# NVIDIA-Merlin/NVTabular

Hardware: AMD Instinct MI355X
Metric: rows/sec + GB/s (Criteo Categorify+FillMissing+Normalize fit+transform, HBM-resident) (higher is better)
Workload: dtype int32 keys -> int64 labels; fp64 moments/normalize; 1 GPU; synthetic Criteo-day0: 26 int32 categorical (Criteo-1TB cardinalities, Zipf) + 13 int32 continuous, nulls as Arrow bitmaps; Categorify + FillMissing + Normalize, fit + transform; rows_per_gpu=45000000, algorithmic_bytes_per_row=624, tie_break=value (count desc, value asc), artifacts=deferred (no parquet I/O inside the timed region)

## Files before the change

nvtabular_amd/csrc/nvt_range_count.hip:

```cpp
#include <cstdio>
#include <cstdlib>
#include <type_traits>

#include "nvt_common.hpp"
#include "nvt_internal.hpp"
#include "nvt_prof.hpp"
#include "nvt_range.hpp"

namespace nvt {

namespace {

constexpr int32_t kEmpty = INT32_MIN;
constexpr int kRpBS = 1024;
constexpr int kRpG = NVT_RANGE_WGS;
constexpr int kRpBinWords = 20480;
constexpr int kRpLine = 16;
constexpr int kRpMaxNbLog2 = 10;
constexpr int kHotSlotsR = NVT_HOT_IMAGE_WORDS;
constexpr int kHotBucketsR = kHotSlotsR / 2;
constexpr int kRpProbe = 512;
#ifndef NVT_RP_MAX_EPOCH
#define NVT_RP_MAX_EPOCH 8
#endif
constexpr unsigned kRpMaxEpoch = NVT_RP_MAX_EPOCH;
#ifndef NVT_RANGE_U
#define NVT_RANGE_U 2
#endif
constexpr unsigned long long kStAgg = 1ull << 62, kStPrefix = 2ull << 62,
                             kStMask = (1ull << 62) - 1ull;

__device__ __forceinline__ uint32_t hot_bucket_r(int32_t key) { return hot_image_bucket(key, kHotBucketsR - 1); }

template <bool PW>
__device__ __forceinline__ uint32_t rp_fine(const RangeMap &map, int32_t key) {
  if constexpr (PW) return map.fine(key);
  else return map.template fine_staged<false>(key);
}


template <int U, int NBL, bool PW>
__global__ __launch_bounds__(kRpBS) void rp_partition_kernel(
    const int32_t *__restrict__ keys, const uint8_t *__restrict__ valid, uint64_t n,
    const int32_t *__restrict__ aux, int nb_log2_rt, uint32_t region_cap, int32_t *__restrict__ regions,
    uint32_t *__restrict__ fills, unsigned *__restrict__ hot_cnt, uint64_t *state,
    unsigned long long *__restrict__ clr_status, unsigned *__restrict__ clr_hist) {
  const int nb_log2 = NBL ? NBL : nb_log2_rt;
  {
    const unsigned nst = (1u << nb_log2) + 8u;
    for (unsigned i = blockIdx.x * kRpBS + threadIdx.x; i < nst; i += kRpG * kRpBS) clr_status[i] = 0ull;
    if (blockIdx.x == kRpG - 1 && threadIdx.x < 256) clr_hist[threadIdx.x] = 0u;
  }
  __shared__ int4 hot[kHotBucketsR];
  __shared__ int32_t bins[kRpBinWords];
  __shared__ unsigned fill[1 << kRpMaxNbLog2], flushed[1 << kRpMaxNbLog2];
  __shared__ unsigned scratch[kWave];
  __shared__ unsigned long long s_nulls, s_sent;
  __shared__ unsigned s_ovf;
  const unsigned NB = 1u << nb_log2, CAP = (unsigned)kRpBinWords >> nb_log2;
  const unsigned g = blockIdx.x, lane = lane_id();
  int32_t fill0 = 0x5A5A5A5A, fill1 = fill0 + 1;
  while (hot_bucket_r(fill1) == hot_bucket_r(fill0)) ++fill1;
  const uint32_t fb0 = hot_bucket_r(fill0);
  for (int i = threadIdx.x; i < kHotBucketsR; i += kRpBS) {
    const int2 k2 = reinterpret_cast<const int2 *>(aux)[i];
    const int32_t fk = (uint32_t)i != fb0 ? fill0 : fill1;
    hot[i] = make_int4(k2.x == kEmpty ? fk : k2.x, k2.y == kEmpty ? fk : k2.y, 0, 0);
  }
  for (unsigned i = threadIdx.x; i < NB; i += kRpBS) {
    fill[i] = 0;
    flushed[i] = 0;
  }
  if (threadIdx.x == 0) {
    s_nulls = 0;
    s_sent = 0;
    s_ovf = 0;
  }
  RangeMap map = load_map(aux);
  __shared__ uint32_t s_pieces[kRpPwWords];
  stage_pieces(map, s_pieces, threadIdx.x, kRpBS);
  __syncthreads();

  const unsigned BPW = NB / (kRpBS / kWave);
  __shared__ unsigned s_epoch[2];
  if (threadIdx.x < 2) s_epoch[threadIdx.x] = 0;
  auto flush_bins = [&](bool all, unsigned parity) {
    {
      const bool owner = lane < BPW;
      const unsigned wave_base = (threadIdx.x / kWave) * BPW;
      const unsigned t = wave_base + (owner ? lane : 0u);
      const unsigned fr = owner ? fill[t] : 0u;
      const unsigned done0 = owner ? flushed[t] : 0u;
      const bool over = fr > CAP;
      const unsigned f = over ? CAP : fr;
      const unsigned nfl = (all || over) ? f : (f / kRpLine) * kRpLine;
      const unsigned padn = over ? ((0u - (done0 + fr)) & (kRpLine - 1u)) : 0u;
      {
        const unsigned long long ob = __ballot(over);
        const unsigned long long hb = __ballot(fr * 2u > CAP);
        if (lane == 0 && (ob | hb))
          atomicAdd(&s_epoch[parity], ((unsigned)__popcll(ob) << 8) | (hb ? 1u : 0u));
      }
      unsigned long long todo = __ballot(nfl > 0);
      const unsigned sub = lane >> 4, l16 = lane & 15;
      while (todo) {
        int sel = -1;
#pragma unroll
        for (unsigned q = 0; q < 4; ++q) {
          const int bit = todo ? (int)__ffsll((long long)todo) - 1 : -1;
          if (todo) todo &= todo - 1;
          sel = (q == sub) ? bit : sel;
        }
        const unsigned src = sel >= 0 ? (unsigned)sel : 0u;
        const unsigned fb = __shfl(f, src, 64), nb_out = __shfl(nfl, src, 64);
        const unsigned done = __shfl(done0, src, 64), frb = __shfl(fr, src, 64), pb = __shfl(padn, src, 64);
        if (sel >= 0) {
          const unsigned bin = wave_base + (unsigned)sel;
          const int32_t *bsrc = bins + bin * CAP;
          const unsigned reach = frb > fb ? done + frb + pb : done + nb_out;
          if (reach > region_cap) {
            if (l16 == 0) atomicOr(&s_ovf, 1u);
          } else {
            int32_t *dst = regions + ((uint64_t)bin * kRpG + g) * region_cap + done;
            for (unsigned u = l16; u < nb_out; u += kRpLine) dst[u] = bsrc[u];
            if (l16 < pb) dst[frb + l16] = kEmpty;
          }
          const unsigned rem = fb - nb_out;
          int32_t keep = 0;
          if (l16 < rem) keep = bsrc[nb_out + l16];
          if (l16 < rem) bins[bin * CAP + l16] = keep;
        }
      }
      if (owner) {
        fill[t] = f - nfl;
        flushed[t] = over ? done0 + fr + padn : done0 + nfl;
      }
    }
  };

  const uint64_t nvec = (n + 3) / 4, nfull = n / 4;
  const uint64_t per = (nvec + kRpG - 1) / kRpG;
  const uint64_t v_lo = (uint64_t)g * per;
  const uint64_t v_hi = v_lo + per < nvec ? v_lo + per : nvec;
  const uint64_t vf_hi = v_hi < nfull ? v_hi : nfull;
  unsigned long long nulls = 0, notvalid = 0;
  unsigned long long empties = 0;
  const uint8_t *vsrc = valid != nullptr ? valid : reinterpret_cast<const uint8_t *>(keys);
  const unsigned vor = valid != nullptr ? 0u : 0xFFu;
  const uint64_t v_last = vf_hi > v_lo ? vf_hi - 1 : 0;
  int4 npack[U];
  unsigned nbyte[U];
  auto issue = [&](uint64_t v0) {
#pragma unroll
    for (int u = 0; u < U; ++u) {
      uint64_t v = v0 + (uint64_t)u * kRpBS;
      v = v < v_last ? v : v_last;
      npack[u] = reinterpret_cast<const int4 *>(keys)[v];
      nbyte[u] = (unsigned)vsrc[v >> 1];
    }
  };
  bool tail_round = false;
  int4 tpack = make_int4(0, 0, 0, 0);
  unsigned tok = 0, tin = 0;
  if (nfull < nvec && nfull >= v_lo && nfull < v_hi) {
    tail_round = true;
    if (threadIdx.x == 0) {
      int32_t kk[4] = {0, 0, 0, 0};
      for (int j = 0; j < 4; ++j) {
        const uint64_t i = nfull * 4 + j;
        if (i < n) {
          tin |= 1u << j;
          if (bit_valid(valid, i)) {
            kk[j] = keys[i];
            tok |= 1u << j;
          }
        }
      }
      tpack = make_int4(kk[0], kk[1], kk[2], kk[3]);
    }
  }
  unsigned R = 1, since = 0, epoch = 0;
  if (vf_hi > v_lo) issue(v_lo + threadIdx.x);
  for (uint64_t v0 = v_lo; v0 < vf_hi || tail_round; v0 += (uint64_t)kRpBS * U) {
    const bool is_tail = !(v0 < vf_hi);
    int32_t kv[4 * U];
    unsigned oks[U], ins[U];
#pragma unroll
    for (int u = 0; u < U; ++u) {
      const uint64_t v = v0 + (uint64_t)u * kRpBS + threadIdx.x;
      const bool present = !is_tail && v < vf_hi;
      kv[4 * u + 0] = npack[u].x;
      kv[4 * u + 1] = npack[u].y;
      kv[4 * u + 2] = npack[u].z;
      kv[4 * u + 3] = npack[u].w;
      oks[u] = present ? (((nbyte[u] | vor) >> (((unsigned)v & 1u) * 4u)) & 0xFu) : 0u;
      ins[u] = present ? 0xFu : 0u;
    }
    if (is_tail) {
      tail_round = false;
      kv[0] = tpack.x;
      kv[1] = tpack.y;
      kv[2] = tpack.z;
      kv[3] = tpack.w;
      oks[0] = tok;
      ins[0] = tin;
    } else {
      issue(v0 + (uint64_t)kRpBS * U + threadIdx.x);
    }
    unsigned pend = 0;
#pragma unroll
    for (int u = 0; u < U; ++u) {
      const unsigned ok = oks[u], in = ins[u];
      nulls += __popc(in & ~ok);
      notvalid += 4u - __popc(ok);
      int32_t kp[4];
      int4 hb[4];
      uint32_t sa[4];
#pragma unroll
      for (int j = 0; j < 4; ++j) {
        const int32_t m = (int32_t)(ok << (31 - j)) >> 31;
        kp[j] = (kv[4 * u + j] & m) | (kEmpty & ~m);
        sa[j] = hot_bucket_r(kp[j]);
      }
#pragma unroll
      for (int j = 0; j < 4; ++j) {
        const int2 kk2 = *reinterpret_cast<const int2 *>(&hot[sa[j]]);
        hb[j].x = kk2.x;
        hb[j].y = kk2.y;
      }
#pragma unroll
      for (int j = 0; j < 4; ++j) {
        const int q = 4 * u + j;
        const int32_t key = kp[j];
        const bool hx = hb[j].x == key, hy = hb[j].y == key;
        const bool hit = hx | hy;
        const bool is_e = key == kEmpty;
        empties += (unsigned)__popcll(__ballot(is_e));
        unsigned *cnt = reinterpret_cast<unsigned *>(&hot[sa[j]]) + (hy ? 3 : 2);
        atomicAdd(hit ? cnt : &scratch[lane], hit ? 1u : 0u);
        pend |= ((!hit & !is_e) ? 1u : 0u) << q;
      }
    }
    if (s_ovf) pend = 0;
#pragma unroll
    for (int q = 0; q < 4 * U; ++q) {
      if ((pend >> q) & 1) {
        const unsigned bkt = rp_fine<PW>(map, kv[q]) >> 14;
        const unsigned pos = atomicAdd(&fill[bkt], 1u);
        if (pos < CAP) {
          bins[bkt * CAP + pos] = kv[q];
        } else {
          const unsigned at = flushed[bkt] + pos;
          if (at < region_cap)
            regions[((uint64_t)bkt * kRpG + g) * region_cap + at] = kv[q];
          else
            atomicOr(&s_ovf, 1u);
        }
      }
    }
    if (++since >= R) {
      __syncthreads();
      flush_bins(false, epoch & 1u);
      if (threadIdx.x == 0) s_epoch[(epoch + 1u) & 1u] = 0;
      __syncthreads();
      const unsigned fl = s_epoch[epoch & 1u];
#ifndef NVT_RP_GROW_DIV
#define NVT_RP_GROW_DIV 16u
#endif
#ifndef NVT_RP_SHRINK_DIV
#define NVT_RP_SHRINK_DIV 4u
#endif
      if ((fl >> 8) > NB / NVT_RP_SHRINK_DIV) R = R > 1u ? R / 2u : 1u;
      else if ((fl >> 8) <= NB / NVT_RP_GROW_DIV) R = R < kRpMaxEpoch ? R * 2u : R;
      ++epoch;
      since = 0;
    }
  }
  __syncthreads();
  flush_bins(true, epoch & 1u);
  __syncthreads();
  for (unsigned b = threadIdx.x; b < NB; b += kRpBS) fills[(uint64_t)b * kRpG + g] = flushed[b];
  for (int i = threadIdx.x; i < kHotBucketsR; i += kRpBS) {
    const int4 hbk = hot[i];
    reinterpret_cast<uint2 *>(hot_cnt + (uint64_t)g * kHotSlotsR)[i] = make_uint2((unsigned)hbk.z, (unsigned)hbk.w);
  }
#pragma unroll
  for (int off = 32; off > 0; off >>= 1) {
    nulls += __shfl_down(nulls, off, 64);
    notvalid += __shfl_down(notvalid, off, 64);
  }
  if (lane == 0) {
    if (nulls) atomicAdd(&s_nulls, nulls);
    const unsigned long long sent = empties - notvalid;
    if (sent) atomicAdd(&s_sent, sent);
  }
  __syncthreads();
  if (threadIdx.x == 0) {
    if (s_nulls) atomicAdd((unsigned long long *)&state[NVT_ST_NULLS], s_nulls);
    if (s_sent) atomicAdd((unsigned long long *)&state[NVT_ST_SENTINEL], s_sent);
    if (s_ovf) atomicOr((unsigned long long *)&state[NVT_ST_OVERFLOW], 1ull | NVT_OVF_REGION);
    if (g == 0) atomicAdd((unsigned long long *)&state[NVT_ST_ROWS], (unsigned long long)n);
  }
}

constexpr int kTotGroups = 16;
__global__ __launch_bounds__(64 * kTotGroups) void hot_totals_kernel(
    const unsigned *__restrict__ hot_cnt, int nblocks, unsigned *__restrict__ hot_tot) {
  __shared__ unsigned part[kTotGroups][64];
  const unsigned l = threadIdx.x & 63, g = threadIdx.x >> 6;
  const unsigned slot = blockIdx.x * 64 + l;
  unsigned t = 0;
#pragma unroll 16
  for (int b = (int)g; b < nblocks; b += kTotGroups) t += hot_cnt[(uint64_t)b * kHotSlotsR + slot];
  part[g][l] = t;
  __syncthreads();
  if (g != 0) return;
  unsigned tot = 0;
#pragma unroll
  for (int q = 0; q < kTotGroups; ++q) tot += part[q][l];
  hot_tot[slot] = tot;
}

template <bool PW>
__global__ __launch_bounds__(kRpBS) void rp_count_kernel(
    const int32_t *__restrict__ regions, const uint32_t *__restrict__ fills, uint32_t region_cap,
    const int32_t *__restrict__ aux, const unsigned *__restrict__ hot_tot, int nb_log2,
    unsigned long long *status, unsigned *ticket, int32_t *__restrict__ out_keys,
    int64_t *__restrict__ out_cnt, uint64_t out_cap, unsigned *cls_hist,
    unsigned long long *__restrict__ range_table, uint64_t *state) {
  constexpr int NSL = kRpSlots + kRpTail;
  constexpr int NW = kRpBS / kWave;
  __shared__ int32_t lkeys[NSL];
  __shared__ unsigned lcnt[NSL];
  __shared__ unsigned run_len[kRpG];
  __shared__ unsigned hist[256];
  __shared__ unsigned wtot[NW];
  __shared__ unsigned lovf, s_b, s_bad, s_mx;
  __shared__ unsigned long long s_base;
  if (threadIdx.x == 0) {
    s_b = atomicAdd(ticket, 1u);
    lovf = 0;
    s_mx = 0;
  }
  for (int i = threadIdx.x; i < NSL; i += kRpBS) {
    lkeys[i] = kEmpty;
    lcnt[i] = 0;
  }
  if (threadIdx.x < 256) hist[threadIdx.x] = 0;
  __syncthreads();
  const unsigned b = s_b, NB = 1u << nb_log2;
  const unsigned lane = lane_id(), w = threadIdx.x / kWave;
  RangeMap map = load_map(aux);
  __shared__ uint32_t s_pieces[kRpPwWords];
  stage_pieces(map, s_pieces, threadIdx.x, kRpBS);
  const bool skip = (state[NVT_ST_OVERFLOW] & 1ull) != 0;
  if (threadIdx.x < kRpG) {
    const unsigned len = fills[(uint64_t)b * kRpG + threadIdx.x];
    run_len[threadIdx.x] = (skip || len > region_cap) ? 0u : len;
  }
  __syncthreads();
  bool failed = skip;
  auto insert_from = [&](int32_t key, unsigned wgt, uint32_t s) {
#pragma unroll 4
    for (int p = 0; p < kRpProbe; ++p, ++s) {
      if (s >= (uint32_t)NSL) break;
      int32_t cur = lkeys[s];
      if (cur == kEmpty) {
        cur = atomicCAS(&lkeys[s], kEmpty, key);
        if (cur == kEmpty) cur = key;
      }
      if (cur == key) {
        atomicAdd(&lcnt[s], wgt);
        return;
      }
    }
    failed = true;
  };
  const unsigned hot_h0 = (unsigned)aux[NVT_RANGE_AUX_HOTSTART + b], hot_h1 = (unsigned)aux[NVT_RANGE_AUX_HOTSTART + b + 1];
  int32_t hot_key0 = kEmpty;
  unsigned hot_tot0 = 0;
  if (hot_h0 + threadIdx.x < hot_h1) {
    const unsigned slot = reinterpret_cast<const unsigned short *>(aux + NVT_RANGE_AUX_HOTORDER)[hot_h0 + threadIdx.x];
    hot_key0 = aux[slot];
    hot_tot0 = hot_tot[slot];
  }
  {
    __shared__ unsigned s_pre[kRpG + 2];
    __shared__ unsigned s_wsum[kRpG / kWave];
    static_assert(kRpG % kWave == 0 && kRpG <= kRpBS, "one thread per run");
    {
      unsigned len = 0, inc = 0;
      if (threadIdx.x < kRpG) {
        len = run_len[threadIdx.x];
        inc = len;
#pragma unroll
        for (int off = 1; off < 64; off <<= 1) {
          const unsigned o = __shfl_up(inc, off, 64);
          if (lane >= (unsigned)off) inc += o;
        }
        if (lane == 63) s_wsum[w] = inc;
      }
      __syncthreads();
      if (threadIdx.x < kRpG) {
        unsigned wb = 0;
        for (unsigned q = 0; q < w; ++q) wb += s_wsum[q];
        s_pre[threadIdx.x] = wb + inc - len;
        if (threadIdx.x == kRpG - 1) s_pre[kRpG] = wb + inc;
      }
    }
    __syncthreads();
    const unsigned *pre = s_pre;
    const unsigned all_keys = pre[kRpG];
    const unsigned share = (all_keys + NW - 1) / NW;
    const unsigned f_lo = w * share < all_keys ? w * share : all_keys;
    const unsigned total = f_lo + share < all_keys ? f_lo + share : all_keys;
    const int32_t *rbase = regions + (uint64_t)b * kRpG * region_cap;
#ifndef NVT_RP_GB
#define NVT_RP_GB 8
#endif
    constexpr int GB = NVT_RP_GB;
    unsigned r = 0;
    {
      const unsigned f = f_lo + lane < all_keys ? f_lo + lane : (all_keys ? all_keys - 1 : 0);
      unsigned lo = 0, hi = kRpG;
      while (hi - lo > 1) {
        const unsigned mid = (lo + hi) >> 1;
        if (pre[mid] <= f) lo = mid; else hi = mid;
      }
      r = lo;
    }
    unsigned r_lo = pre[r], r_hi = pre[r + 1];
    for (unsigned f0 = f_lo; f0 < total && !failed; f0 += GB * kWave) {
      int32_t kk[GB];
#pragma unroll
      for (int u = 0; u < GB; ++u) {
        const unsigned f = f0 + u * kWave + lane;
        kk[u] = kEmpty;
        if (f < total) {
          while (f >= r_hi) {
            ++r;
            r_lo = r_hi;
            r_hi = pre[r + 1];
          }
          kk[u] = rbase[(uint64_t)r * region_cap + (f - r_lo)];
        }
      }
      uint32_t hs[GB];
      int32_t cur[GB];
#pragma unroll
      for (int u = 0; u < GB; ++u) hs[u] = rp_fine<PW>(map, kk[u]) & (kRpSlots - 1);
#pragma unroll
      for (int u = 0; u < GB; ++u) cur[u] = lkeys[hs[u]];
#pragma unroll
      for (int u = 0; u < GB; ++u) {
        if (cur[u] == kEmpty && kk[u] != kEmpty) {
          cur[u] = atomicCAS(&lkeys[hs[u]], kEmpty, kk[u]);
          cur[u] = cur[u] == kEmpty ? kk[u] : cur[u];
        }
      }
      unsigned todo = 0;
#pragma unroll
      for (int u = 0; u < GB; ++u) {
        if (kk[u] == kEmpty) continue;
        if (cur[u] == kk[u])
          atomicAdd(&lcnt[hs[u]], 1u);
        else
          todo |= 1u << u;
      }
      int32_t wkey = 0;
      uint32_t ws = 0;
      int wp = 0;
      bool walking = false;
      while (true) {
        if (!walking && todo) {
          const int u = (int)__ffs((int)todo) - 1;
          wkey = kk[0];
          ws = hs[0];
#pragma unroll
          for (int q = 1; q < GB; ++q) {
            wkey = u == q ? kk[q] : wkey;
            ws = u == q ? hs[q] : ws;
          }
          todo &= todo - 1u;
          ++ws;
          wp = 1;
          walking = true;
        }
        if (!__any(walking)) break;
        if (walking) {
          if (ws >= (uint32_t)NSL || wp >= kRpProbe) {
            failed = true;
            walking = false;
          } else {
            int32_t c = lkeys[ws];
            if (c == kEmpty) {
              c = atomicCAS(&lkeys[ws], kEmpty, wkey);
              if (c == kEmpty) c = wkey;
            }
            if (c == wkey) {
              atomicAdd(&lcnt[ws], 1u);
              walking = false;
            } else {
              ++ws;
              ++wp;
            }
          }
        }
      }
    }
  }
  {
    if (hot_key0 != kEmpty && hot_tot0 > 0 && !failed)
      insert_from(hot_key0, hot_tot0, rp_fine<PW>(map, hot_key0) & (kRpSlots - 1));
    const unsigned short *order = reinterpret_cast<const unsigned short *>(aux + NVT_RANGE_AUX_HOTORDER);
    for (unsigned jx = hot_h0 + threadIdx.x + kRpBS; jx < hot_h1; jx += kRpBS) {
      const unsigned slot = order[jx];
      const int32_t key = aux[slot];
      const unsigned tot = hot_tot[slot];
      if (key != kEmpty && tot > 0 && !failed) insert_from(key, tot, rp_fine<PW>(map, key) & (kRpSlots - 1));
    }
  }
  if (failed) atomicOr(&lovf, 1u);
  __syncthreads();
  if (threadIdx.x == 0)
    s_bad = (lovf != 0 ||
             (__hip_atomic_load(&state[NVT_ST_OVERFLOW], __ATOMIC_RELAXED,
                                __HIP_MEMORY_SCOPE_AGENT) & 1ull))
                ? 1u : 0u;
  __syncthreads();
  const bool bad = s_bad != 0;
  const unsigned long long sent_rows = b == 0 ? state[NVT_ST_SENTINEL] : 0ull;
  const unsigned extra = sent_rows > 0 ? 1u : 0u;
  constexpr int ITER = (NSL + kRpBS - 1) / kRpBS;
  unsigned mine = 0;
  for (int it = 0; it < ITER; ++it) {
    const int i = it * kRpBS + (int)threadIdx.x;
    const bool occ = i < NSL && lkeys[i] != kEmpty;
    mine += (unsigned)__popcll(__ballot(occ));
  }
  if (lane == 0) wtot[w] = mine;
  __syncthreads();
  unsigned E = extra;
  for (int q = 0; q < NW; ++q) E += wtot[q];
  const bool full = E > (unsigned)(kRpSlots / 4 * 3);
  if (bad || full) E = 0;
  if (w == 0) {
    unsigned long long excl = 0;
    if (lane == 0)
      __hip_atomic_store(&status[b], (b == 0 ? kStPrefix : kStAgg) | (unsigned long long)E,
                         __ATOMIC_RELAXED, __HIP_MEMORY_SCOPE_AGENT);
    if (b > 0) {
      int top = (int)b - 1;
      while (true) {
        const int idx = top - (int)lane;
        unsigned long long v = kStPrefix;
        if (idx >= 0) {
          do {
            v = __hip_atomic_load(&status[idx], __ATOMIC_RELAXED, __HIP_MEMORY_SCOPE_AGENT);
#ifndef NVT_RP_SLEEP
#define NVT_RP_SLEEP 1
#endif
            if ((v >> 62) == 0) __builtin_amdgcn_s_sleep(NVT_RP_SLEEP);
          } while ((v >> 62) == 0);
        }
        const unsigned long long isp = __ballot((v >> 62) == 2);
        const int first = isp ? (int)__ffsll((long long)isp) - 1 : 64;
        unsigned long long add = ((int)lane <= first) ? (v & kStMask) : 0ull;
#pragma unroll
        for (int off = 32; off > 0; off >>= 1) add += __shfl_down(add, off, 64);
        excl += __shfl(add, 0, 64);
        if (isp) break;
        top -= 64;
      }
      if (lane == 0)
        __hip_atomic_store(&status[b], kStPrefix | (excl + E), __ATOMIC_RELAXED,
                           __HIP_MEMORY_SCOPE_AGENT);
    }
    if (lane == 0) s_base = excl;
  }
  __syncthreads();
  const unsigned long long base = s_base;
  if (b == NB - 1 && threadIdx.x == 0) {
    if (base + E > out_cap) {
      atomicOr((unsigned long long *)&state[NVT_ST_OVERFLOW], 2ull);
      state[NVT_ST_NEED] = base + E;
    } else {
      state[NVT_ST_OCCUPIED] = base + E;
    }
  }
  if (bad || full) {
    if (threadIdx.x == 0 && (lovf != 0 || full))
      atomicOr((unsigned long long *)&state[NVT_ST_OVERFLOW],
               1ull | (lovf != 0 ? NVT_OVF_PROBE : 0ull) | (full ? NVT_OVF_FULL : 0ull));
    return;
  }
  if (base + E > out_cap) return;
  if (extra && threadIdx.x == 0) {
    out_keys[base] = kEmpty;
    out_cnt[base] = (int64_t)sent_rows;
    const unsigned cls = sent_rows < 255 ? (unsigned)sent_rows : 255u;
    atomicAdd(&hist[cls], 1u);
    unsigned long long *gm = reinterpret_cast<unsigned long long *>(&state[NVT_ST_MAXCOUNT]);
    atomicMax(gm, sent_rows);
  }
  __shared__ unsigned occ_pre[ITER * NW];
  __shared__ unsigned occ_wsum[8];
  for (int it = 0; it < ITER; ++it) {
    const int i = it * kRpBS + (int)threadIdx.x;
    const bool occ = i < NSL && lkeys[i] != kEmpty;
    const unsigned c = (unsigned)__popcll(__ballot(occ));
    if (lane == 0) occ_pre[it * NW + w] = c;
  }
  __syncthreads();
  {
    constexpr int NG = ITER * NW;
    constexpr int SW = (NG + kWave - 1) / kWave;
    unsigned v = 0, inc = 0;
    if (w < (unsigned)SW) {
      v = threadIdx.x < (unsigned)NG ? occ_pre[threadIdx.x] : 0u;
      inc = v;
#pragma unroll
      for (int off = 1; off < 64; off <<= 1) {
        const unsigned o = __shfl_up(inc, off, 64);
        if (lane >= (unsigned)off) inc += o;
      }
      if (lane == 63) occ_wsum[w] = inc;
    }
    __syncthreads();
    if (w < (unsigned)SW && threadIdx.x < (unsigned)NG) {
      unsigned wb = 0;
      for (unsigned q = 0; q < w; ++q) wb += occ_wsum[q];
      occ_pre[threadIdx.x] = extra + wb + inc - v;
    }
    __syncthreads();
  }
  unsigned mx = 0;
  for (int it = 0; it < ITER; ++it) {
    const int i = it * kRpBS + (int)threadIdx.x;
    const int32_t k = i < NSL ? lkeys[i] : kEmpty;
    const bool occ = k != kEmpty;
    unsigned long long dump = kEncEmptySlot;
    const unsigned long long bal = __ballot(occ);
    const unsigned front = occ_pre[it * NW + w];
    if (occ) {
      const unsigned p_i = front + (unsigned)__popcll(bal & ((1ull << lane) - 1ull));
      unsigned rank = 0;
      int s = i;
      while (true) {
        int32_t o[4];
#pragma unroll
        for (int q = 0; q < 4; ++q) o[q] = s - 1 - q >= 0 ? lkeys[s - 1 - q] : kEmpty;
        int run = 0;
        bool open = true;
#pragma unroll
        for (int q = 0; q < 4; ++q) {
          open = open && o[q] != kEmpty;
          run += open ? 1 : 0;
          rank += (open && o[q] < k) ? 1u : 0u;
        }
        s -= run;
        if (run < 4) break;
      }
      int e = i + 1;
      while (true) {
        int32_t o[4];
#pragma unroll
        for (int q = 0; q < 4; ++q) o[q] = e + q < NSL ? lkeys[e + q] : kEmpty;
        int run = 0;
        bool open = true;
#pragma unroll
        for (int q = 0; q < 4; ++q) {
          open = open && o[q] != kEmpty;
          run += open ? 1 : 0;
          rank += (open && o[q] < k) ? 1u : 0u;
        }
        e += run;
        if (run < 4) break;
      }
      const uint64_t pos = base + p_i - (unsigned)(i - s) + rank;
      const unsigned c = lcnt[i];
      out_keys[pos] = k;
      out_cnt[pos] = (int64_t)c;
      atomicAdd(&hist[c < 255u ? c : 255u], 1u);
      mx = c > mx ? c : mx;
      dump = ((unsigned long long)(uint32_t)pos << 32) | (uint32_t)k;
    }
    if (range_table != nullptr && i < NSL) range_table[(uint64_t)b * NSL + i] = dump;
  }
#pragma unroll
  for (int off = 32; off > 0; off >>= 1) {
    const unsigned o = __shfl_down(mx, off, 64);
    mx = o > mx ? o : mx;
  }
  if (lane == 0 && mx > 0) atomicMax(&s_mx, mx);
  if (range_table != nullptr && b == NB - 1 && threadIdx.x < kRpGuard)
    range_table[(uint64_t)NB * NSL + threadIdx.x] = kEncEmptySlot;
  __syncthreads();
  if (threadIdx.x == 0 && s_mx > 0)
    atomicMax(reinterpret_cast<unsigned long long *>(&state[NVT_ST_MAXCOUNT]), (unsigned long long)s_mx);
  if (threadIdx.x < 256) {
    const unsigned h = hist[threadIdx.x];
    if (h) atomicAdd(&cls_hist[threadIdx.x], h);
    if (threadIdx.x == 255 && h)
      atomicAdd((unsigned long long *)&state[NVT_ST_BIG], (unsigned long long)h);
  }
}

inline uint64_t al16(uint64_t x) { return (x + 15) & ~15ull; }

}

uint32_t range_region_cap(uint64_t n, int nb_log2) {
  const uint64_t rows_per_wg = (n + kRpG - 1) / kRpG;
  const uint64_t c = 2 * (rows_per_wg >> nb_log2) + 64;
  return (uint32_t)((c + kRpLine - 1) / kRpLine * kRpLine);
}

struct RangeWs {
  int32_t *regions;
  uint32_t *fills;
  unsigned *hot_cnt, *hot_tot;
  unsigned long long *status;
  unsigned *ticket;
};

uint64_t range_ws_layout(uint64_t n, int nb_log2, char *base, RangeWs *ws) {
  uint64_t off = 0;
  auto take = [&](uint64_t bytes) {
    char *p = base ? base + off : nullptr;
    off += al16(bytes);
    return p;
  };
  RangeWs w;
  const uint64_t NB = 1ull << nb_log2;
  w.regions = (int32_t *)take(NB * kRpG * range_region_cap(n, nb_log2) * 4);
  w.fills = (uint32_t *)take(NB * kRpG * 4);
  w.hot_cnt = (unsigned *)take((uint64_t)kRpG * kHotSlotsR * 4);
  w.hot_tot = (unsigned *)take((uint64_t)kHotSlotsR * 4);
  w.status = (unsigned long long *)take(NB * 8 + 64);
  w.ticket = (unsigned *)(w.status ? (char *)w.status + NB * 8 : nullptr);
  if (ws) *ws = w;
  return off;
}

uint64_t range_count_ws_bytes(uint64_t n, int nb_log2) {
  return range_ws_layout(n, nb_log2, nullptr, nullptr);
}

int range_count_i32(const int32_t *keys, const uint8_t *valid, uint64_t n, int nb_log2, void *wsp,
                    int32_t *aux, int32_t *out_keys, int64_t *out_cnt, uint64_t out_cap,
                    void *range_table, uint64_t *state, hipStream_t s, bool pieces) {
  NVT_CHECK_ARG(nb_log2 >= 6 && nb_log2 <= kRpMaxNbLog2, "range path: 64 .. 1024 buckets");
  NVT_CHECK_ARG(aux != nullptr, "range path: the column needs its aux block (hot_image)");
  NVT_PROF("dense_count_r9", n * 4, s);
  RangeWs w;
  range_ws_layout(n, nb_log2, (char *)wsp, &w);
  const unsigned NB = 1u << nb_log2;
  const uint32_t cap = range_region_cap(n, nb_log2);
  unsigned *hist = (unsigned *)(aux + NVT_RANGE_AUX_HIST);
#define NVT_RP_PART(NBL)                                                                            \
  do {                                                                                              \
    if (pieces)                                                                                     \
      rp_partition_kernel<NVT_RANGE_U, NBL, true><<<kRpG, kRpBS, 0, s>>>(                           \
          keys, valid, n, aux, nb_log2, cap, w.regions, w.fills, w.hot_cnt, state, w.status, hist); \
    else                                                                                            \
      rp_partition_kernel<NVT_RANGE_U, NBL, false><<<kRpG, kRpBS, 0, s>>>(                          \
          keys, valid, n, aux, nb_log2, cap, w.regions, w.fills, w.hot_cnt, state, w.status, hist); \
  } while (0)
  if (nb_log2 == 8) NVT_RP_PART(8);
  else if (nb_log2 == 9) NVT_RP_PART(9);
  else if (nb_log2 == 10) NVT_RP_PART(10);
  else NVT_RP_PART(0);
#undef NVT_RP_PART
  NVT_CHECK_LAUNCH();
  hot_totals_kernel<<<kHotSlotsR / 64, 64 * kTotGroups, 0, s>>>(w.hot_cnt, kRpG, w.hot_tot);
  NVT_CHECK_LAUNCH();
  if (pieces)
    rp_count_kernel<true><<<NB, kRpBS, 0, s>>>(w.regions, w.fills, cap, aux, w.hot_tot, nb_log2, w.status,
                                               w.ticket, out_keys, out_cnt, out_cap,
                                               (unsigned *)(aux + NVT_RANGE_AUX_HIST),
                                               (unsigned long long *)range_table, state);
  else
    rp_count_kernel<false><<<NB, kRpBS, 0, s>>>(w.regions, w.fills, cap, aux, w.hot_tot, nb_log2, w.status,
                                                w.ticket, out_keys, out_cnt, out_cap,
                                                (unsigned *)(aux + NVT_RANGE_AUX_HIST),
                                                (unsigned long long *)range_table, state);
  NVT_CHECK_LAUNCH();
  return NVT_OK;
}

}
```

Before: 4.966 billion rows/s.

## Overlap local rank computation with decoupled look-back in range count kernel

```diff
diff --git a/nvtabular_amd/csrc/nvt_range_count.hip b/nvtabular_amd/csrc/nvt_range_count.hip
--- a/nvtabular_amd/csrc/nvt_range_count.hip
+++ b/nvtabular_amd/csrc/nvt_range_count.hip
@@ -330,11 +330,11 @@
     unsigned long long *__restrict__ range_table, uint64_t *state) {
   constexpr int NSL = kRpSlots + kRpTail;
   constexpr int NW = kRpBS / kWave;
-  __shared__ int32_t lkeys[NSL];
+  constexpr int kRpWalkPad = 3;
+  __shared__ int32_t lkeys[NSL + kRpWalkPad];
   __shared__ unsigned lcnt[NSL];
   __shared__ unsigned run_len[kRpG];
   __shared__ unsigned hist[256];
-  __shared__ unsigned wtot[NW];
   __shared__ unsigned lovf, s_b, s_bad, s_mx;
   __shared__ unsigned long long s_base;
   if (threadIdx.x == 0) {
@@ -532,18 +532,51 @@
   const unsigned long long sent_rows = b == 0 ? state[NVT_ST_SENTINEL] : 0ull;
   const unsigned extra = sent_rows > 0 ? 1u : 0u;
   constexpr int ITER = (NSL + kRpBS - 1) / kRpBS;
-  unsigned mine = 0;
+  constexpr int NG = ITER * NW;
+  constexpr int SW = (NG + kWave - 1) / kWave;
+  __shared__ unsigned long long occ_bits[NG];
+  __shared__ unsigned occ_pre[NG];
+  __shared__ unsigned occ_wsum[SW];
   for (int it = 0; it < ITER; ++it) {
     const int i = it * kRpBS + (int)threadIdx.x;
     const bool occ = i < NSL && lkeys[i] != kEmpty;
-    mine += (unsigned)__popcll(__ballot(occ));
-  }
-  if (lane == 0) wtot[w] = mine;
-  __syncthreads();
+    const unsigned long long bal = __ballot(occ);
+    if (lane == 0) {
+      occ_bits[it * NW + w] = bal;
+      occ_pre[it * NW + w] = (unsigned)__popcll(bal);
+    }
+  }
+  __syncthreads();
+  {
+    unsigned v = 0, inc = 0;
+    if (w < (unsigned)SW) {
+      v = threadIdx.x < (unsigned)NG ? occ_pre[threadIdx.x] : 0u;
+      inc = v;
+#pragma unroll
+      for (int off = 1; off < 64; off <<= 1) {
+        const unsigned o = __shfl_up(inc, off, 64);
+        if (lane >= (unsigned)off) inc += o;
+      }
+      if (lane == 63) occ_wsum[w] = inc;
+    }
+    __syncthreads();
+    if (w < (unsigned)SW && threadIdx.x < (unsigned)NG) {
+      unsigned wb = 0;
+      for (unsigned q = 0; q < w; ++q) wb += occ_wsum[q];
+      occ_pre[threadIdx.x] = extra + wb + inc - v;
+    }
+    __syncthreads();
+  }
   unsigned E = extra;
-  for (int q = 0; q < NW; ++q) E += wtot[q];
+  for (int q = 0; q < SW; ++q) E += occ_wsum[q];
   const bool full = E > (unsigned)(kRpSlots / 4 * 3);
   if (bad || full) E = 0;
+  constexpr int RT = kRpBS - kWave;
+  constexpr int RITER = (NSL + RT - 1) / RT;
+  constexpr unsigned kNoEntry = 0xFFFFu;
+  static_assert(kRpSlots / 4 * 3 + 1 < (int)kNoEntry && RITER % 2 == 0, "positions are packed in 16-bit pairs");
+  unsigned lpos[RITER / 2];
+  const int rt = (int)threadIdx.x - kWave;
   if (w == 0) {
     unsigned long long excl = 0;
     if (lane == 0)
@@ -577,6 +610,33 @@
                            __HIP_MEMORY_SCOPE_AGENT);
     }
     if (lane == 0) s_base = excl;
+  } else if (!(bad || full)) {
+#pragma unroll
+    for (int j = 0; j < RITER; ++j) {
+      const int i = j * RT + rt;
+      const int32_t k = i < NSL ? lkeys[i] : kEmpty;
+      unsigned p = kNoEntry;
+      if (k != kEmpty) {
+        const uint32_t h = rp_fine<PW>(map, k) & (kRpSlots - 1);
+        unsigned wi = h >> 6;
+        const unsigned long long win = occ_bits[wi];
+        p = occ_pre[wi] + (unsigned)__popcll(win & ((1ull << (h & 63u)) - 1ull));
+        unsigned long long z = ~win & (~0ull << (h & 63u));
+        while (z == 0ull) z = ~occ_bits[++wi];
+        const int e = (int)(wi * 64u) + (int)__ffsll((long long)z) - 1;
+#pragma unroll 1
+        for (int s = (int)h; s < e; s += 4) {
+          int32_t o[4];
+#pragma unroll
+          for (int q = 0; q < 4; ++q) o[q] = lkeys[s + q];
+          const int left = e - s;
+#pragma unroll
+          for (int q = 0; q < 4; ++q) p += (q < left && o[q] < k) ? 1u : 0u;
+        }
+      }
+      if (j & 1) lpos[j / 2] |= p << 16;
+      else lpos[j / 2] = p;
+    }
   }
   __syncthreads();
   const unsigned long long base = s_base;
@@ -603,89 +663,26 @@
     unsigned long long *gm = reinterpret_cast<unsigned long long *>(&state[NVT_ST_MAXCOUNT]);
     atomicMax(gm, sent_rows);
   }
-  __shared__ unsigned occ_pre[ITER * NW];
-  __shared__ unsigned occ_wsum[8];
-  for (int it = 0; it < ITER; ++it) {
-    const int i = it * kRpBS + (int)threadIdx.x;
-    const bool occ = i < NSL && lkeys[i] != kEmpty;
-    const unsigned c = (unsigned)__popcll(__ballot(occ));
-    if (lane == 0) occ_pre[it * NW + w] = c;
-  }
-  __syncthreads();
-  {
-    constexpr int NG = ITER * NW;
-    constexpr int SW = (NG + kWave - 1) / kWave;
-    unsigned v = 0, inc = 0;
-    if (w < (unsigned)SW) {
-      v = threadIdx.x < (unsigned)NG ? occ_pre[threadIdx.x] : 0u;
-      inc = v;
-#pragma unroll
-      for (int off = 1; off < 64; off <<= 1) {
-        const unsigned o = __shfl_up(inc, off, 64);
-        if (lane >= (unsigned)off) inc += o;
-      }
-      if (lane == 63) occ_wsum[w] = inc;
-    }
-    __syncthreads();
-    if (w < (unsigned)SW && threadIdx.x < (unsigned)NG) {
-      unsigned wb = 0;
-      for (unsigned q = 0; q < w; ++q) wb += occ_wsum[q];
-      occ_pre[threadIdx.x] = extra + wb + inc - v;
-    }
-    __syncthreads();
-  }
   unsigned mx = 0;
-  for (int it = 0; it < ITER; ++it) {
-    const int i = it * kRpBS + (int)threadIdx.x;
-    const int32_t k = i < NSL ? lkeys[i] : kEmpty;
-    const bool occ = k != kEmpty;
-    unsigned long long dump = kEncEmptySlot;
-    const unsigned long long bal = __ballot(occ);
-    const unsigned front = occ_pre[it * NW + w];
-    if (occ) {
-      const unsigned p_i = front + (unsigned)__popcll(bal & ((1ull << lane) - 1ull));
-      unsigned rank = 0;
-      int s = i;
-      while (true) {
-        int32_t o[4];
-#pragma unroll
-        for (int q = 0; q < 4; ++q) o[q] = s - 1 - q >= 0 ? lkeys[s - 1 - q] : kEmpty;
-        int run = 0;
-        bool open = true;
-#pragma unroll
-        for (int q = 0; q < 4; ++q) {
-          open = open && o[q] != kEmpty;
-          run += open ? 1 : 0;
-          rank += (open && o[q] < k) ? 1u : 0u;
-        }
-        s -= run;
-        if (run < 4) break;
-      }
-      int e = i + 1;
-      while (true) {
-        int32_t o[4];
-#pragma unroll
-        for (int q = 0; q < 4; ++q) o[q] = e + q < NSL ? lkeys[e + q] : kEmpty;
-        int run = 0;
-        bool open = true;
-#pragma unroll
-        for (int q = 0; q < 4; ++q) {
-          open = open && o[q] != kEmpty;
-          run += open ? 1 : 0;
-          rank += (open && o[q] < k) ? 1u : 0u;
-        }
-        e += run;
-        if (run < 4) break;
-      }
-      const uint64_t pos = base + p_i - (unsigned)(i - s) + rank;
-      const unsigned c = lcnt[i];
-      out_keys[pos] = k;
-      out_cnt[pos] = (int64_t)c;
-      atomicAdd(&hist[c < 255u ? c : 255u], 1u);
-      mx = c > mx ? c : mx;
-      dump = ((unsigned long long)(uint32_t)pos << 32) | (uint32_t)k;
-    }
-    if (range_table != nullptr && i < NSL) range_table[(uint64_t)b * NSL + i] = dump;
+  if (w != 0) {
+#pragma unroll
+    for (int j = 0; j < RITER; ++j) {
+      const int i = j * RT + rt;
+      if (i >= NSL) break;
+      const unsigned p = (j & 1) ? lpos[j / 2] >> 16 : lpos[j / 2] & 0xFFFFu;
+      unsigned long long dump = kEncEmptySlot;
+      if (p != kNoEntry) {
+        const int32_t k = lkeys[i];
+        const unsigned c = lcnt[i];
+        const uint64_t pos = base + p;
+        out_keys[pos] = k;
+        out_cnt[pos] = (int64_t)c;
+        atomicAdd(&hist[c < 255u ? c : 255u], 1u);
+        mx = c > mx ? c : mx;
+        dump = ((unsigned long long)(uint32_t)pos << 32) | (uint32_t)k;
+      }
+      if (range_table != nullptr) range_table[(uint64_t)b * NSL + i] = dump;
+    }
   }
 #pragma unroll
   for (int off = 32; off > 0; off >>= 1) {
```

Result: faster. 5.029 billion rows/s (median of 6 runs) (+1.3%).
